# yihua7/NeRF-Texture

Measured on AMD Instinct MI355X. Metric: ray-samples/s (train), higher is better.
Workload: dtype f16

## Files before the change

nerf-texture_amd/csrc/common.hpp:

```cpp
#pragma once

#include <hip/hip_runtime.h>
#include <hip/hip_fp16.h>
#include <stdint.h>

#include <cstdarg>
#include <cstdio>

#include "../../include/nerftex_hip.h"

namespace nerftex {

void set_error(const char* fmt, ...);
void clear_error();

inline hipStream_t as_stream(void* s) { return reinterpret_cast<hipStream_t>(s); }

inline int check_launch(const char* what) {
    hipError_t e = hipGetLastError();
    if (e != hipSuccess) {
        set_error("%s: HIP launch failed: %s", what, hipGetErrorString(e));
        return NERFTEX_ERR_HIP;
    }
    return NERFTEX_OK;
}

#define NERFTEX_HIP_TRY(expr, what)                                                   \
    do {                                                                              \
        hipError_t _e = (expr);                                                       \
        if (_e != hipSuccess) {                                                       \
            ::nerftex::set_error("%s: %s", what, hipGetErrorString(_e));              \
            return NERFTEX_ERR_HIP;                                                   \
        }                                                                             \
    } while (0)

template <typename T>
constexpr T div_up(T a, T b) { return (a + b - 1) / b; }

inline int device_cus() {
    static int cus[16] = {0};
    int dev = 0;
    if (hipGetDevice(&dev) != hipSuccess || dev < 0 || dev >= 16) return 256;
    if (cus[dev] == 0) {
        hipDeviceProp_t prop;
        cus[dev] = (hipGetDeviceProperties(&prop, dev) == hipSuccess && prop.multiProcessorCount > 0) ? prop.multiProcessorCount : 256;
    }
    return cus[dev];
}

enum Knob {
    kKnobGridFwd,
    kKnobGridBwd,
    kKnobGridBwdSweep,
    kKnobGridBwdItems,
    kKnobGridBwdSlice,
    kKnobGridBwdNoMerge,
    kKnobGridBwdProbe,
    kKnobMarch,
    kKnobMarchSerial,
    kKnobFfmlpWgPerCu,
    kKnobFfmlpBwdSplit,
    kKnobMarchLean,
    kKnobFfmlpBwdTr,
    kKnobGridBwdStage,
    kKnobCompositeKeep,
    kKnobCount
};
extern long g_knobs[kKnobCount];
inline long knob(Knob k) { return g_knobs[k]; }

extern int g_profile_mode;
constexpr int kTimeAny = 1, kTimeGrid = 2;
void profile_begin(const char* name, hipStream_t st, int* slot);
void profile_end(hipStream_t st, int slot);
struct KernelTimer {
    hipStream_t st;
    int slot = -1;
    KernelTimer(const char* name, hipStream_t s, int group = kTimeAny) : st(s) {
        if (g_profile_mode == 1 || (g_profile_mode == 2 && group == kTimeGrid)) profile_begin(name, s, &slot);
    }
    ~KernelTimer() { if (slot >= 0) profile_end(st, slot); }
};

using half_t = _Float16;
typedef _Float16 half2_t __attribute__((ext_vector_type(2)));
typedef _Float16 half4_t __attribute__((ext_vector_type(4)));
typedef _Float16 half8_t __attribute__((ext_vector_type(8)));
typedef float float2_t __attribute__((ext_vector_type(2)));
typedef float float4_t __attribute__((ext_vector_type(4)));
typedef float float16_t __attribute__((ext_vector_type(16)));

constexpr int kWave = 64;

__host__ __device__ __forceinline__ uint32_t unit_rows(uint32_t code, uint32_t count) {
    if (!(code >> 31)) return code;
    const uint32_t F = (code >> 24) & 127u, N = code & 0xffffffu;
    const uint32_t q = F * N / (count ? count : 1u);
    return q < F ? F : (q > 8u * F ? 8u * F : q);
}
__device__ __forceinline__ uint32_t live_rows(uint32_t B, const int32_t* __restrict__ units_dev, uint32_t rows_per_unit) {
    if (!units_dev) return B;
    const uint32_t n = (uint32_t)units_dev[0];
    return min(B, n * unit_rows(rows_per_unit, n));
}
__device__ __forceinline__ bool slot_unused(const float* __restrict__ dirs, size_t row) { return dirs[row * 3] > 1e29f; }

}
```

nerf-texture_amd/csrc/raymarching.hip:

```cpp
#include "common.hpp"
#include "step_loss.hpp"
#include "workspace.hpp"

#include <cstdlib>
#include <type_traits>

#pragma clang fp contract(off)

namespace nerftex {
namespace {

constexpr float kSqrt3 = 1.7320508075688772f;
constexpr float kRPi = 0.3183098861837907f;
constexpr uint32_t kBlock = 256;
constexpr uint32_t kRayBlock = 64;

struct Pcg32 {
    uint64_t state, inc;
    static constexpr uint64_t kMult = 0x5851f42d4c957f2dULL;

    __host__ __device__ explicit Pcg32(uint64_t initstate, uint64_t initseq = 1) {
        state = 0;
        inc = (initseq << 1u) | 1u;
        next_uint();
// ... 212 lines not shown
    near_out = near;
    far_out = far;
}

__global__ __launch_bounds__(kBlock) void near_far_kernel(const float* __restrict__ rays_o, const float* __restrict__ rays_d,
                                                          const float* __restrict__ aabb, uint32_t N, float min_near,
                                                          float* __restrict__ nears, float* __restrict__ fars) {
    const uint32_t n = blockIdx.x * blockDim.x + threadIdx.x;
    if (n >= N) return;
    float near, far;
    near_far_of(rays_o, rays_d, aabb, min_near, (size_t)n, near, far);
    nears[n] = near;
    fars[n] = far;
}

__global__ __launch_bounds__(kBlock) void polar_kernel(const float* __restrict__ rays_o, const float* __restrict__ rays_d,
                                                       float radius, uint32_t N, float* __restrict__ coords) {
    const uint32_t n = blockIdx.x * blockDim.x + threadIdx.x;
    if (n >= N) return;
    const float ox = rays_o[3 * (size_t)n], oy = rays_o[3 * (size_t)n + 1], oz = rays_o[3 * (size_t)n + 2];
    const float dx = rays_d[3 * (size_t)n], dy = rays_d[3 * (size_t)n + 1], dz = rays_d[3 * (size_t)n + 2];
    const float A = fmaf(dz, dz, fmaf(dy, dy, dx * dx));
    const float Bh = fmaf(oz, dz, fmaf(oy, dy, ox * dx));
    const float Cc = fmaf(-radius, radius, fmaf(oz, oz, fmaf(oy, oy, ox * ox)));
    const float t = (-Bh + sqrtf(fmaf(Bh, Bh, -(A * Cc)))) / A;
    const float x = fmaf(t, dx, ox), y = fmaf(t, dy, oy), z = fmaf(t, dz, oz);
    const float theta = atan2f(sqrtf(fmaf(z, z, x * x)), y);
    const float phi = atan2f(z, x);
    coords[2 * (size_t)n] = fmaf(2 * theta, kRPi, -1.0f);
    coords[2 * (size_t)n + 1] = phi * kRPi;
}

__global__ __launch_bounds__(kBlock) void morton3D_kernel(const int* __restrict__ coords, uint32_t N, int* __restrict__ indices) {
    const uint32_t n = blockIdx.x * blockDim.x + threadIdx.x;
    if (n >= N) return;
    indices[n] = (int)morton3D((uint32_t)coords[3 * (size_t)n], (uint32_t)coords[3 * (size_t)n + 1], (uint32_t)coords[3 * (size_t)n + 2]);
}

__global__ __launch_bounds__(kBlock) void morton3D_invert_kernel(const int* __restrict__ indices, uint32_t N, int* __restrict__ coords) {
    const uint32_t n = blockIdx.x * blockDim.x + threadIdx.x;
    if (n >= N) return;
    const int ind = indices[n];
    coords[3 * (size_t)n + 0] = (int)morton3D_invert((uint32_t)(ind >> 0));
    coords[3 * (size_t)n + 1] = (int)morton3D_invert((uint32_t)(ind >> 1));
    coords[3 * (size_t)n + 2] = (int)morton3D_invert((uint32_t)(ind >> 2));
}

__global__ __launch_bounds__(kBlock) void packbits_kernel(const float* __restrict__ grid, uint32_t N, float thresh,
                                                          uint8_t* __restrict__ bitfield) {
    const uint32_t n = blockIdx.x * blockDim.x + threadIdx.x;
    if (n >= N) return;
    const float4_t a = *reinterpret_cast<const float4_t*>(grid + (size_t)n * 8);
    const float4_t b = *reinterpret_cast<const float4_t*>(grid + (size_t)n * 8 + 4);
    uint32_t bits = 0;
#pragma unroll
    for (int i = 0; i < 4; i++) {
        bits |= (a[i] > thresh) ? (1u << i) : 0u;
        bits |= (b[i] > thresh) ? (1u << (4 + i)) : 0u;
    }
    bitfield[n] = (uint8_t)bits;
}

__device__ __forceinline__ float ray_t0(const Dda& s, float near, uint32_t perturb, uint32_t n, uint64_t seed) {
    float t0 = near;
    if (perturb) {
        Pcg32 rng(seed);
        rng.advance((uint64_t)n);
        t0 = fmaf(s.dt_min, rng.next_float(), t0);
    }
    return t0;
}

#ifndef NERFTEX_MC_RAYS
#define NERFTEX_MC_RAYS 32
#endif
constexpr uint32_t kMcRays = NERFTEX_MC_RAYS;
static_assert(kRayBlock % kMcRays == 0, "the expand pass adds whole count-pass totals per 64-ray block");
constexpr uint32_t kMcSeg = 128;
constexpr uint32_t kMcSub = 32;
constexpr uint32_t kMcThreads = kMcRays * kMcSub;
constexpr uint32_t kMcPer = kMcSeg / kMcSub;
constexpr uint32_t kMcTPitch = kMcRays + 1;
constexpr uint32_t kMcJPitch = kMcSeg + 4;

template <bool LEAN>
__global__ __launch_bounds__(kMcThreads, LEAN ? 8 : 4) void march_count_parallel_kernel(const float* __restrict__ rays_o, const float* __restrict__ rays_d,
                                                                         const uint8_t* __restrict__ grid, float bound, float dt_gamma,
                                                                         uint32_t max_steps, uint32_t N, uint32_t C, uint32_t H,
                                                                         const float* __restrict__ nears, const float* __restrict__ fars,
                                                                         int* __restrict__ rays, const int* __restrict__ counter,
                                                                         uint32_t* __restrict__ ws, uint32_t perturb, float* __restrict__ tlog,
                                                                         const float* __restrict__ aabb, float min_near,
                                                                         float* __restrict__ nears_w, float* __restrict__ fars_w) {
    __shared__ float s_T[kMcSeg * kMcTPitch];
    __shared__ uint8_t s_jump[kMcRays * kMcJPitch];
    __shared__ uint8_t s_vis[kMcRays * kMcJPitch];
    __shared__ uint32_t s_cnt[kMcRays];
    __shared__ uint32_t s_full[kMcRays];
    __shared__ uint32_t s_base[kMcRays];
    __shared__ uint32_t s_live;

    const uint32_t tid = threadIdx.x;
    const uint32_t own = tid, n_own = blockIdx.x * kMcRays + own;
    const bool owner = tid < kMcRays && n_own < N;
    const uint32_t r2 = tid / kMcSub, sub = tid % kMcSub, n2 = blockIdx.x * kMcRays + r2;
    const bool has2 = n2 < N;
    float near2 = 0.0f, far2 = 0.0f;
    if (has2) {
        if (aabb) near_far_of(rays_o, rays_d, aabb, min_near, (size_t)n2, near2, far2);
        else far2 = fars[n2];
    }
    const Dda s2(rays_o + 3 * (size_t)(has2 ? n2 : 0), rays_d + 3 * (size_t)(has2 ? n2 : 0), bound, dt_gamma, max_steps, C, H, grid, far2);
    float* log_row2 = tlog + (size_t)(has2 ? n2 : 0) * max_steps;

    float t_next = 0.0f, far = 0.0f, pending_tt = 0.0f;
    bool pending = false, done = true;
    uint32_t num = 0;
    if (owner) {
        float near;
        if (aabb) {
            near_far_of(rays_o, rays_d, aabb, min_near, (size_t)n_own, near, far);
            nears_w[n_own] = near;
            fars_w[n_own] = far;
        } else {
            far = fars[n_own];
            near = nears[n_own];
        }
        t_next = ray_t0(s2, near, perturb, n_own, 42);
        done = !(t_next < far);
    }
    const float dt_min = s2.dt_lo, dt_max = s2.dt_max;

    for (;;) {
        if (tid == 0) s_live = 0;
        for (uint32_t i = tid; i < kMcRays * kMcJPitch / 4; i += kMcThreads) reinterpret_cast<uint32_t*>(s_vis)[i] = 0u;
        __syncthreads();
        if (tid < kMcRays) {
            uint32_t cnt = 0;
            if (owner && !done) {
                float t = t_next;
                while (cnt < kMcSeg) {
                    const float t0 = t;
                    const float t1 = t0 + __builtin_amdgcn_fmed3f(t0 * dt_gamma, dt_min, dt_max);
                    const float t2 = t1 + __builtin_amdgcn_fmed3f(t1 * dt_gamma, dt_min, dt_max);
                    const float t3 = t2 + __builtin_amdgcn_fmed3f(t2 * dt_gamma, dt_min, dt_max);
                    s_T[(cnt + 0) * kMcTPitch + own] = t0;
                    s_T[(cnt + 1) * kMcTPitch + own] = t1;
                    s_T[(cnt + 2) * kMcTPitch + own] = t2;
                    s_T[(cnt + 3) * kMcTPitch + own] = t3;
                    if (!(t3 < far)) {
                        cnt += (t0 < far ? 1u : 0u) + (t1 < far ? 1u : 0u) + (t2 < far ? 1u : 0u);
                        t = far;
                        break;
                    }
                    cnt += 4;
                    t = t3 + __builtin_amdgcn_fmed3f(t3 * dt_gamma, dt_min, dt_max);
                }
                t_next = t;
                atomicOr(&s_live, 1u);
            }
            s_cnt[own] = cnt;
            s_full[own] = (owner && !done && cnt == kMcSeg && t_next < far) ? 1u : 0u;
            s_base[own] = num;
        }
        __syncthreads();
        if (s_live == 0) break;

        {
            const uint32_t cnt = s_cnt[r2];
            Dda::Cell cell[kMcPer];
            uint8_t occ_byte[kMcPer];
#pragma unroll
            for (uint32_t i = 0; i < kMcPer; i++) {
                const uint32_t k = sub + kMcSub * i;
                occ_byte[i] = 0;
                cell[i] = Dda::Cell{};
                if (k < cnt) {
                    const uint32_t index = s2.locate(s_T[k * kMcTPitch + r2], cell[i]);
                    occ_byte[i] = grid[index >> 3];
                }
            }
#pragma unroll
            for (uint32_t i = 0; i < kMcPer; i++) {
                const uint32_t k = sub + kMcSub * i;
                if (k < cnt) {
                    uint32_t jump = 0;
                    if (!((occ_byte[i] >> (cell[i].packed >> 29)) & 1u)) {
                        const float t = s_T[k * kMcTPitch + r2];
                        const float tt = s2.exit_of(t, cell[i]);
                        uint32_t j = k + 1;
                        for (;;) {
                            uint32_t c = 0;
#pragma unroll
                            for (uint32_t q = 0; q < 4; q++) c += (j + q < cnt && s_T[(j + q) * kMcTPitch + r2] < tt) ? 1u : 0u;
                            j += c;
                            if (c < 4) break;
                        }
                        jump = j - k;
                    }
                    s_jump[r2 * kMcJPitch + k] = (uint8_t)jump;
                }
            }
        }
        __syncthreads();

        if (owner && !done) {
            const uint32_t cnt = s_cnt[own];
            const bool full = s_full[own] != 0;
            const uint8_t* jr = s_jump + own * kMcJPitch;
            uint8_t* vr = s_vis + own * kMcJPitch;
            uint32_t k = 0;
            if (pending) {
                while (k < cnt && s_T[k * kMcTPitch + own] < pending_tt) k++;
                pending = k == cnt && full;
            }
            uint32_t last_skip = 0xffffffffu;
            while (k < cnt && num < max_steps) {
                const uint32_t j = jr[k];
                const uint32_t sample = j == 0 ? 1u : 0u;
                vr[k] = (uint8_t)sample;
                num += sample;
                last_skip = (j != 0 && k + j == cnt) ? k : last_skip;
                k += j + sample;
            }
            if (full && last_skip != 0xffffffffu && k == cnt && num < max_steps) {
                Dda::Cell c;
                const float t = s_T[last_skip * kMcTPitch + own];
                const Dda so(rays_o + 3 * (size_t)n_own, rays_d + 3 * (size_t)n_own, bound, dt_gamma, max_steps, C, H, grid, far);
                (void)so.locate(t, c);
                pending_tt = so.exit_of(t, c);
                pending = true;
            }
            if (!full || num >= max_steps) done = true;
        }
        __syncthreads();

        {
            uint32_t mine = 0;
            uint32_t flags = 0;
#pragma unroll
            for (uint32_t i = 0; i < kMcPer; i++) {
                const uint32_t k = sub * kMcPer + i;
                const uint32_t v = s_vis[r2 * kMcJPitch + k];
                flags |= v << i;
                mine += v;
            }
            uint32_t incl = mine;
#pragma unroll
            for (int off = 1; off < (int)kMcSub; off <<= 1) {
                const uint32_t o = __shfl_up(incl, off, kMcSub);
                if ((int)sub >= off) incl += o;
            }
            uint32_t at = s_base[r2] + incl - mine;
            if (has2 && flags) {
#pragma unroll
                for (uint32_t i = 0; i < kMcPer; i++)
                    if ((flags >> i) & 1u) log_row2[at++] = s_T[(sub * kMcPer + i) * kMcTPitch + r2];
            }
        }
        __syncthreads();
    }

    if (owner) rays[3 * (size_t)n_own + 2] = (int)num;
    if (tid < kWave) {
        const uint32_t wsum = wave_sum(tid < kMcRays ? num : 0u);
        if (tid == 0) {
            ws[1 + blockIdx.x] = wsum;
            if (blockIdx.x == 0) ws[0] = aabb ? 0u : (uint32_t)counter[0];
        }
    }
}

__global__ __launch_bounds__(kRayBlock) void march_count_kernel(const float* __restrict__ rays_o, const float* __restrict__ rays_d,
                                                             const uint8_t* __restrict__ grid, float bound, float dt_gamma,
                                                             uint32_t max_steps, uint32_t N, uint32_t C, uint32_t H,
                                                             const float* __restrict__ nears, const float* __restrict__ fars,
                                                             int* __restrict__ rays, const int* __restrict__ counter,
                                                             uint32_t* __restrict__ ws, uint32_t perturb, float* __restrict__ tlog) {
    __shared__ uint32_t wave_tot[kRayBlock / kWave];
    const uint32_t n = blockIdx.x * blockDim.x + threadIdx.x;
    uint32_t num_steps = 0;
    if (n < N) {
        const Dda s(rays_o + 3 * (size_t)n, rays_d + 3 * (size_t)n, bound, dt_gamma, max_steps, C, H, grid, fars[n]);
        float t = ray_t0(s, nears[n], perturb, n, 42);
        float x, y, z, dt;
        float* log_row = tlog ? tlog + (size_t)n * max_steps : nullptr;
        while (t < s.far && num_steps < max_steps) {
            if (s.step(t, x, y, z, dt)) {
                if (log_row) log_row[num_steps] = t;
                num_steps++;
                t += dt;
            }
        }
        rays[3 * (size_t)n + 2] = (int)num_steps;
    }
    const uint32_t wsum = wave_sum(num_steps);
    if ((threadIdx.x & (kWave - 1)) == 0) wave_tot[threadIdx.x / kWave] = wsum;
    __syncthreads();
    if (threadIdx.x == 0) {
        uint32_t tot = 0;
#pragma unroll
        for (uint32_t i = 0; i < kRayBlock / kWave; i++) tot += wave_tot[i];
        ws[1 + blockIdx.x] = tot;
        if (blockIdx.x == 0) ws[0] = (uint32_t)counter[0];
    }
}

template <bool WITH_TS>
__global__ __launch_bounds__(kRayBlock) void march_write_kernel(const float* __restrict__ rays_o, const float* __restrict__ rays_d,
                                                             const uint8_t* __restrict__ grid, float bound, float dt_gamma,
                                                             uint32_t max_steps, uint32_t N, uint32_t C, uint32_t H, uint32_t M,
                                                             const float* __restrict__ nears, const float* __restrict__ fars,
                                                             float* __restrict__ xyzs, float* __restrict__ dirs,
                                                             float* __restrict__ deltas, float* __restrict__ rays_ts,
                                                             int* __restrict__ rays, int* __restrict__ counter,
                                                             const uint32_t* __restrict__ ws, uint32_t perturb) {
    __shared__ uint32_t red[kRayBlock / kWave];
    __shared__ uint32_t wave_tot[kRayBlock / kWave];
    const uint32_t n = blockIdx.x * blockDim.x + threadIdx.x;
    const uint32_t lane = threadIdx.x & (kWave - 1), wid = threadIdx.x / kWave;

    uint32_t part = 0;
    for (uint32_t j = threadIdx.x; j < blockIdx.x; j += kRayBlock) part += ws[1 + j];
    part = wave_sum(part);
    if (lane == 0) red[wid] = part;

    const uint32_t num_steps = n < N ? (uint32_t)rays[3 * (size_t)n + 2] : 0u;
    const uint32_t incl = wave_inclusive_scan(num_steps);
    if (lane == kWave - 1) wave_tot[wid] = incl;
    __syncthreads();
    uint32_t before = ws[0];
#pragma unroll
    for (uint32_t i = 0; i < kRayBlock / kWave; i++) {
        before += red[i];
        if (i < wid) before += wave_tot[i];
    }
    const uint32_t point_index = before + incl - num_steps;

    if (blockIdx.x == gridDim.x - 1 && threadIdx.x == kRayBlock - 1) {
        counter[0] = (int)(point_index + num_steps);
        counter[1] = counter[1] + (int)N;
    }
    if (n >= N) return;

    rays[3 * (size_t)n] = (int)n;
    rays[3 * (size_t)n + 1] = (int)point_index;
    if (num_steps == 0) return;
    if (point_index + num_steps >= M) return;
// ... 645 lines not shown
    const float t_old = n < n_alive ? rays_t_old[n] : -1.0f;
    const bool keep = n < n_alive && t_old >= 0;
    const uint64_t mask = __ballot(keep);
    const uint32_t rank = (uint32_t)__popcll(mask & ((1ull << lane) - 1ull));
    if (lane == 0) wave_tot[wid] = (uint32_t)__popcll(mask);
    __syncthreads();
    uint32_t before = ws[0];
    uint32_t block_total = 0;
#pragma unroll
    for (uint32_t i = 0; i < kBlock / kWave; i++) {
        before += red[i];
        if (i < wid) before += wave_tot[i];
        block_total += wave_tot[i];
    }
    if (keep) {
        const uint32_t dst = before + rank;
        rays_alive[dst] = rays_alive_old[n];
        rays_t[dst] = t_old;
    }
    if (blockIdx.x == gridDim.x - 1 && threadIdx.x == 0) {
        uint32_t prior = ws[0];
#pragma unroll
        for (uint32_t i = 0; i < kBlock / kWave; i++) prior += red[i];
        uint32_t survivors = prior + block_total;
        if (steps_done != nullptr) {
            const uint32_t done = steps_done[0];
            if (done >= max_steps) survivors = 0u;
            else steps_done[0] = done + unit_rows(n_step_code, survivors);
        }
        alive_counter[0] = (int)survivors;
        if (host_mirror != nullptr) __hip_atomic_store(host_mirror, (int)survivors, __ATOMIC_RELAXED, __HIP_MEMORY_SCOPE_SYSTEM);
    }
}

inline dim3 grid_for(uint32_t n) { return dim3(div_up(n, kBlock)); }
inline dim3 ray_grid_for(uint32_t n) { return dim3(div_up(n, kRayBlock)); }

__global__ __launch_bounds__(kBlock) void zero_words_kernel(uint32_t* __restrict__ a, size_t na, uint32_t* __restrict__ b, size_t nb) {
    for (size_t i = (size_t)blockIdx.x * kBlock + threadIdx.x; i < na + nb; i += (size_t)gridDim.x * kBlock) {
        if (i < na) a[i] = 0u;
        else b[i - na] = 0u;
    }
}

template <bool WITH_TS>
int march_train_impl(const float* rays_o, const float* rays_d, const uint8_t* grid, float bound, float dt_gamma,
                     uint32_t max_steps, uint32_t N, uint32_t C, uint32_t H, uint32_t M, const float* nears, const float* fars,
                     float* xyzs, float* dirs, float* deltas, float* rays_ts, int32_t* rays, int32_t* counter, uint32_t perturb,
                     void* stream, const float* aabb = nullptr, float min_near = 0.0f) {
    clear_error();
    if (N == 0) return NERFTEX_OK;
    if (C == 0 || C > 16) {
        set_error("march_rays_train: cascade count C=%u out of range", C);
        return NERFTEX_ERR_INVALID;
    }
    const uint32_t nblocks = div_up(N, kRayBlock);
    const size_t head = (sizeof(uint32_t) * (1 + (size_t)div_up(N, kMcRays)) + 255) / 256 * 256;
    const size_t log_bytes = sizeof(float) * (size_t)N * max_steps;
    const long force = knob(kKnobMarch);
    const bool use_log = force ? force == 2 : (log_bytes <= ((size_t)1 << 30));
    char* base = static_cast<char*>(workspace(kWsMarch, head + (use_log ? log_bytes : 0), as_stream(stream)));
    if (!base) return NERFTEX_ERR_HIP;
    uint32_t* ws = reinterpret_cast<uint32_t*>(base);
    float* tlog = use_log ? reinterpret_cast<float*>(base + head) : nullptr;
    hipStream_t st = as_stream(stream);
    const bool parallel_count = use_log && H <= 256 && !knob(kKnobMarchSerial);
    if (aabb && !parallel_count) {
        {
            KernelTimer kt("near_far_kernel", st);
            hipLaunchKernelGGL(near_far_kernel, grid_for(N), dim3(kBlock), 0, st, rays_o, rays_d, aabb, N, min_near, const_cast<float*>(nears),
                               const_cast<float*>(fars));
        }
        {
            KernelTimer kt("zero_words_kernel", st);
            hipLaunchKernelGGL(zero_words_kernel, dim3(1024), dim3(kBlock), 0, st, reinterpret_cast<uint32_t*>(xyzs), (size_t)M * 8,
                               reinterpret_cast<uint32_t*>(counter), (size_t)2);
        }
        int rc0 = check_launch("march_rays_train_fresh(prologue)");
        if (rc0 != NERFTEX_OK) return rc0;
        aabb = nullptr;
    }
    if (parallel_count) {
        KernelTimer kt("march_count_parallel_kernel", st);
        if (knob(kKnobMarchLean))
            hipLaunchKernelGGL(march_count_parallel_kernel<true>, dim3(div_up(N, kMcRays)), dim3(kMcThreads), 0, st, rays_o, rays_d, grid, bound, dt_gamma,
                               max_steps, N, C, H, nears, fars, rays, counter, ws, perturb, tlog, aabb, min_near, const_cast<float*>(nears),
                               const_cast<float*>(fars));
        else
            hipLaunchKernelGGL(march_count_parallel_kernel<false>, dim3(div_up(N, kMcRays)), dim3(kMcThreads), 0, st, rays_o, rays_d, grid, bound, dt_gamma,
                               max_steps, N, C, H, nears, fars, rays, counter, ws, perturb, tlog, aabb, min_near, const_cast<float*>(nears),
                               const_cast<float*>(fars));
    } else {
        KernelTimer kt("march_count_kernel", st);
        hipLaunchKernelGGL(march_count_kernel, dim3(nblocks), dim3(kRayBlock), 0, st, rays_o, rays_d, grid, bound, dt_gamma, max_steps, N,
                           C, H, nears, fars, rays, counter, ws, perturb, tlog);
    }
    int rc = check_launch("march_rays_train(count)");
    if (rc != NERFTEX_OK) return rc;
    if (use_log) {
        {
            KernelTimer kt("march_expand_kernel", st);
            hipLaunchKernelGGL((march_expand_kernel<WITH_TS>), dim3(nblocks), dim3(kExpandThreads), 0, st, rays_o, rays_d, bound, dt_gamma, max_steps, N, C, H, M,
                               nears, xyzs, dirs, deltas, rays_ts, rays, counter, ws, perturb, tlog, parallel_count ? kRayBlock / kMcRays : 1u,
                               parallel_count ? div_up(N, kMcRays) : nblocks, aabb ? 1u : 0u);
        }
        return check_launch("march_rays_train(expand)");
    }
    {
        KernelTimer kt("march_write_kernel", st);
        hipLaunchKernelGGL((march_write_kernel<WITH_TS>), dim3(nblocks), dim3(kRayBlock), 0, st, rays_o, rays_d, grid, bound, dt_gamma,
                           max_steps, N, C, H, M, nears, fars, xyzs, dirs, deltas, rays_ts, rays, counter, ws, perturb);
    }
    return check_launch("march_rays_train(write)");
}

}
}

using namespace nerftex;

extern "C" int nerftex_near_far_from_aabb(const float* rays_o, const float* rays_d, const float* aabb, uint32_t N, float min_near,
                                          float* nears, float* fars, void* stream) {
    clear_error();
    if (N == 0) return NERFTEX_OK;
    {
        KernelTimer kt("near_far_kernel", as_stream(stream));
        hipLaunchKernelGGL(near_far_kernel, grid_for(N), dim3(kBlock), 0, as_stream(stream), rays_o, rays_d, aabb, N, min_near, nears, fars);
    }
    return check_launch("near_far_from_aabb");
}

extern "C" int nerftex_polar_from_ray(const float* rays_o, const float* rays_d, float radius, uint32_t N, float* coords, void* stream) {
    clear_error();
    if (N == 0) return NERFTEX_OK;
    {
        KernelTimer kt("polar_kernel", as_stream(stream));
        hipLaunchKernelGGL(polar_kernel, grid_for(N), dim3(kBlock), 0, as_stream(stream), rays_o, rays_d, radius, N, coords);
    }
    return check_launch("polar_from_ray");
}

extern "C" int nerftex_morton3D(const int32_t* coords, uint32_t N, int32_t* indices, void* stream) {
    clear_error();
    if (N == 0) return NERFTEX_OK;
    {
        KernelTimer kt("morton3D_kernel", as_stream(stream));
        hipLaunchKernelGGL(morton3D_kernel, grid_for(N), dim3(kBlock), 0, as_stream(stream), coords, N, indices);
    }
    return check_launch("morton3D");
}

extern "C" int nerftex_morton3D_invert(const int32_t* indices, uint32_t N, int32_t* coords, void* stream) {
    clear_error();
    if (N == 0) return NERFTEX_OK;
    {
        KernelTimer kt("morton3D_invert_kernel", as_stream(stream));
        hipLaunchKernelGGL(morton3D_invert_kernel, grid_for(N), dim3(kBlock), 0, as_stream(stream), indices, N, coords);
    }
    return check_launch("morton3D_invert");
}

extern "C" int nerftex_packbits(const float* grid, uint32_t N, float density_thresh, uint8_t* bitfield, void* stream) {
    clear_error();
    if (N == 0) return NERFTEX_OK;
    {
        KernelTimer kt("packbits_kernel", as_stream(stream));
        hipLaunchKernelGGL(packbits_kernel, grid_for(N), dim3(kBlock), 0, as_stream(stream), grid, N, density_thresh, bitfield);
    }
    return check_launch("packbits");
}

extern "C" int nerftex_march_rays_train(const float* rays_o, const float* rays_d, const uint8_t* grid, float bound, float dt_gamma,
                                        uint32_t max_steps, uint32_t N, uint32_t C, uint32_t H, uint32_t M, const float* nears,
                                        const float* fars, float* xyzs, float* dirs, float* deltas, int32_t* rays, int32_t* counter,
// ... 296 lines not shown
```

nerf-texture_amd/csrc/runtime.hip:

```cpp
#include "common.hpp"
#include "workspace.hpp"

#include <atomic>

#include <cstdlib>
#include <cstring>
#include <map>
#include <mutex>
#include <string>
#include <vector>

namespace nerftex {

static thread_local char g_err[512] = {0};

void set_error(const char* fmt, ...) {
    va_list ap;
    va_start(ap, fmt);
    vsnprintf(g_err, sizeof(g_err), fmt, ap);
    va_end(ap);
}

void clear_error() { g_err[0] = 0; }

long g_knobs[kKnobCount] = {0};
namespace {
const char* const kKnobNames[kKnobCount] = {"grid_fwd", "grid_bwd", "grid_bwd_sweep", "grid_bwd_items", "grid_bwd_slice", "grid_bwd_nomerge",
                                            "grid_bwd_probe", "march", "march_serial", "ffmlp_wg_per_cu",
                                            "ffmlp_bwd_split", "march_lean", "ffmlp_bwd_tr", "grid_bwd_stage", "composite_keep"};
int knob_index(const char* name, size_t n) {
    for (int k = 0; k < kKnobCount; k++)
        if (strlen(kKnobNames[k]) == n && strncmp(kKnobNames[k], name, n) == 0) return k;
    return -1;
}
struct KnobInit {
    KnobInit() {
        auto env = [](const char* n) { const char* v = getenv(n); return v ? v : ""; };
        const char* v;
        v = env("NERFTEX_GRID_FWD"); g_knobs[kKnobGridFwd] = v[0] == 'p' ? 1 : v[0] == 'l' ? 2 : 0;
        v = env("NERFTEX_GRID_BWD"); g_knobs[kKnobGridBwd] = v[0] == 'a' ? 1 : v[0] == 'o' ? 2 : 0;
        g_knobs[kKnobGridBwdSweep] = env("NERFTEX_GRID_BWD_ALGO")[0] == 's';
        g_knobs[kKnobGridBwdItems] = atol(env("NERFTEX_GRID_BWD_ITEMS"));
        g_knobs[kKnobGridBwdSlice] = atol(env("NERFTEX_GRID_BWD_SLICE"));
        g_knobs[kKnobGridBwdNoMerge] = getenv("NERFTEX_GRID_BWD_NOMERGE") != nullptr;
        v = env("NERFTEX_MARCH"); g_knobs[kKnobMarch] = v[0] == 'r' ? 1 : v[0] == 'l' ? 2 : 0;
        g_knobs[kKnobMarchSerial] = env("NERFTEX_MARCH_COUNT")[0] == 's';
        g_knobs[kKnobFfmlpWgPerCu] = atol(env("NERFTEX_FFMLP_WG_PER_CU"));
        g_knobs[kKnobFfmlpBwdSplit] = env("NERFTEX_FFMLP_BWD")[0] == 's';
        for (const char* p = env("NERFTEX_TUNE"); *p;) {
            const char* eq = strchr(p, '=');
            if (!eq) break;
            const int k = knob_index(p, (size_t)(eq - p));
            if (k >= 0) g_knobs[k] = atol(eq + 1);
            const char* c = strchr(eq, ',');
            if (!c) break;
            p = c + 1;
        }
    }
} g_knob_init;
}

namespace {
constexpr int kMaxDevices = 16;
struct Slot { void* ptr = nullptr; size_t bytes = 0; };
struct SlotSet { Slot slot[kWsSlots]; };
std::map<hipStream_t, SlotSet> g_ws[kMaxDevices];
const hipStream_t kCaptureSet = reinterpret_cast<hipStream_t>(~(uintptr_t)0);
std::vector<void*> g_retired;
std::mutex g_ws_mutex;
}

std::atomic<unsigned> g_ws_touched{0};
thread_local int t_capture_set = 0;

void* workspace(WorkspaceSlot slot, size_t bytes, hipStream_t stream) {
    g_ws_touched.fetch_or(1u << (unsigned)slot, std::memory_order_relaxed);
    int dev = 0;
    if (hipGetDevice(&dev) != hipSuccess || dev < 0 || dev >= kMaxDevices) {
        set_error("workspace: bad device");
        return nullptr;
    }
    hipStreamCaptureStatus cap = hipStreamCaptureStatusNone;
    if (hipStreamIsCapturing(stream, &cap) == hipSuccess && cap != hipStreamCaptureStatusNone)
        stream = reinterpret_cast<hipStream_t>(reinterpret_cast<uintptr_t>(kCaptureSet) - (uintptr_t)t_capture_set);
    std::lock_guard<std::mutex> lock(g_ws_mutex);
    Slot& s = g_ws[dev][stream].slot[slot];
    if (s.bytes < bytes) {
        if (s.ptr) g_retired.push_back(s.ptr);
        s.ptr = nullptr;
        s.bytes = 0;
        size_t want = bytes < (1u << 20) ? (1u << 20) : bytes + bytes / 2;
        hipStreamCaptureMode mode = hipStreamCaptureModeRelaxed;
        (void)hipThreadExchangeStreamCaptureMode(&mode);
        const hipError_t err = hipMalloc(&s.ptr, want);
        (void)hipThreadExchangeStreamCaptureMode(&mode);
        if (err != hipSuccess) {
            set_error("workspace: hipMalloc(%zu) failed", want);
            s.ptr = nullptr;
            return nullptr;
        }
        s.bytes = want;
        static const int poison = [] { const char* v = getenv("NERFTEX_POISON_WORKSPACE"); return v && *v ? atoi(v) : -1; }();
        if (poison >= 0) {
            (void)hipThreadExchangeStreamCaptureMode(&mode);
            (void)hipMemset(s.ptr, poison & 255, want);
            (void)hipThreadExchangeStreamCaptureMode(&mode);
        }
    }
    return s.ptr;
}

bool peek_workspace(int slot, hipStream_t stream, void** ptr, size_t* bytes) {
// ... 147 lines not shown
```

Baseline: 909.8 million.

## Parallelize march count skip-chain walk with pointer jumping across ray sub-lanes

Replaces the serial per-ray owner walk over the jump table in the parallel march-count kernel with a pointer-jumping pass run by the 32 lanes assigned to each ray, synchronized at wave level. The pending-skip offset is computed with a shuffle reduction, cell exit times are carried in registers instead of being re-located, and sample offsets come from ballot/popcount. This removes a serial loop and two block barriers per segment. In exchange it adds several rounds of LDS traffic per segment, and it adds a probe knob that can skip phases for timing.

```diff
diff --git a/nerf-texture_amd/csrc/common.hpp b/nerf-texture_amd/csrc/common.hpp
--- a/nerf-texture_amd/csrc/common.hpp
+++ b/nerf-texture_amd/csrc/common.hpp
@@ -64,6 +64,7 @@
     kKnobFfmlpBwdTr,
     kKnobGridBwdStage,
     kKnobCompositeKeep,
+    kKnobMarchCountProbe,
     kKnobCount
 };
 extern long g_knobs[kKnobCount];
diff --git a/nerf-texture_amd/csrc/raymarching.hip b/nerf-texture_amd/csrc/raymarching.hip
--- a/nerf-texture_amd/csrc/raymarching.hip
+++ b/nerf-texture_amd/csrc/raymarching.hip
@@ -318,6 +318,15 @@
 constexpr uint32_t kMcPer = kMcSeg / kMcSub;
 constexpr uint32_t kMcTPitch = kMcRays + 1;
 constexpr uint32_t kMcJPitch = kMcSeg + 4;
+constexpr uint32_t kMcRounds = 7;
+static_assert((1u << kMcRounds) >= kMcSeg && kMcSeg <= 255, "a path is covered by the rounds; member indices fit a byte");
+static_assert(kMcSub == 32 && kWave == 64, "a ray is one half of a wave in phases 2-4 (ballot halves, wave-level ordering of LDS)");
+
+__device__ __forceinline__ void wave_lds_order() {
+    __builtin_amdgcn_fence(__ATOMIC_RELEASE, "wavefront");
+    __builtin_amdgcn_wave_barrier();
+    __builtin_amdgcn_fence(__ATOMIC_ACQUIRE, "wavefront");
+}
 
 template <bool LEAN>
 __global__ __launch_bounds__(kMcThreads, LEAN ? 8 : 4) void march_count_parallel_kernel(const float* __restrict__ rays_o, const float* __restrict__ rays_d,
@@ -327,19 +336,21 @@
                                                                          int* __restrict__ rays, const int* __restrict__ counter,
                                                                          uint32_t* __restrict__ ws, uint32_t perturb, float* __restrict__ tlog,
                                                                          const float* __restrict__ aabb, float min_near,
-                                                                         float* __restrict__ nears_w, float* __restrict__ fars_w) {
+                                                                         float* __restrict__ nears_w, float* __restrict__ fars_w, const uint32_t probe) {
     __shared__ float s_T[kMcSeg * kMcTPitch];
-    __shared__ uint8_t s_jump[kMcRays * kMcJPitch];
-    __shared__ uint8_t s_vis[kMcRays * kMcJPitch];
+    __shared__ uint32_t s_next[kMcRays * kMcJPitch / 4];
+    __shared__ uint32_t s_mark[kMcRays * kMcJPitch / 4];
     __shared__ uint32_t s_cnt[kMcRays];
     __shared__ uint32_t s_full[kMcRays];
-    __shared__ uint32_t s_base[kMcRays];
+    __shared__ uint32_t s_num[kMcRays];
+    __shared__ uint32_t s_done[kMcRays];
     __shared__ uint32_t s_live;
 
     const uint32_t tid = threadIdx.x;
     const uint32_t own = tid, n_own = blockIdx.x * kMcRays + own;
     const bool owner = tid < kMcRays && n_own < N;
     const uint32_t r2 = tid / kMcSub, sub = tid % kMcSub, n2 = blockIdx.x * kMcRays + r2;
+    const uint32_t half = tid & 32u;
     const bool has2 = n2 < N;
     float near2 = 0.0f, far2 = 0.0f;
     if (has2) {
@@ -348,62 +359,88 @@
     }
     const Dda s2(rays_o + 3 * (size_t)(has2 ? n2 : 0), rays_d + 3 * (size_t)(has2 ? n2 : 0), bound, dt_gamma, max_steps, C, H, grid, far2);
     float* log_row2 = tlog + (size_t)(has2 ? n2 : 0) * max_steps;
-
-    float t_next = 0.0f, far = 0.0f, pending_tt = 0.0f;
-    bool pending = false, done = true;
+    uint32_t* const next_w = s_next + r2 * (kMcJPitch / 4) + sub;
+    uint32_t* const mark_w = s_mark + r2 * (kMcJPitch / 4) + sub;
+    uint8_t* const next_b = reinterpret_cast<uint8_t*>(s_next + r2 * (kMcJPitch / 4));
+    uint8_t* const mark_b = reinterpret_cast<uint8_t*>(s_mark + r2 * (kMcJPitch / 4));
+
+    float t_next = 0.0f, far = 0.0f;
+    if (tid < kMcRays) {
+        bool done = true;
+        if (owner) {
+            float near;
+            if (aabb) {
+                near_far_of(rays_o, rays_d, aabb, min_near, (size_t)n_own, near, far);
+                nears_w[n_own] = near;
+                fars_w[n_own] = far;
+            } else {
+                far = fars[n_own];
+                near = nears[n_own];
+            }
+            t_next = ray_t0(s2, near, perturb, n_own, 42);
+            done = !(t_next < far);
+        }
+        s_done[own] = done ? 1u : 0u;
+        s_num[own] = 0u;
+    }
+    const float dt_min = s2.dt_lo, dt_max = s2.dt_max;
+    float pending_tt = 0.0f;
+    bool pending = false;
     uint32_t num = 0;
-    if (owner) {
-        float near;
-        if (aabb) {
-            near_far_of(rays_o, rays_d, aabb, min_near, (size_t)n_own, near, far);
-            nears_w[n_own] = near;
-            fars_w[n_own] = far;
-        } else {
-            far = fars[n_own];
-            near = nears[n_own];
-        }
-        t_next = ray_t0(s2, near, perturb, n_own, 42);
-        done = !(t_next < far);
-    }
-    const float dt_min = s2.dt_lo, dt_max = s2.dt_max;
 
     for (;;) {
         if (tid == 0) s_live = 0;
-        for (uint32_t i = tid; i < kMcRays * kMcJPitch / 4; i += kMcThreads) reinterpret_cast<uint32_t*>(s_vis)[i] = 0u;
-        __syncthreads();
         if (tid < kMcRays) {
             uint32_t cnt = 0;
-            if (owner && !done) {
+            const bool run = owner && s_done[own] == 0;
+            if (run) {
                 float t = t_next;
-                while (cnt < kMcSeg) {
+#pragma unroll 2
+                for (uint32_t k = 0; k < kMcSeg; k += 4) {
                     const float t0 = t;
                     const float t1 = t0 + __builtin_amdgcn_fmed3f(t0 * dt_gamma, dt_min, dt_max);
                     const float t2 = t1 + __builtin_amdgcn_fmed3f(t1 * dt_gamma, dt_min, dt_max);
                     const float t3 = t2 + __builtin_amdgcn_fmed3f(t2 * dt_gamma, dt_min, dt_max);
-                    s_T[(cnt + 0) * kMcTPitch + own] = t0;
-                    s_T[(cnt + 1) * kMcTPitch + own] = t1;
-                    s_T[(cnt + 2) * kMcTPitch + own] = t2;
-                    s_T[(cnt + 3) * kMcTPitch + own] = t3;
-                    if (!(t3 < far)) {
-                        cnt += (t0 < far ? 1u : 0u) + (t1 < far ? 1u : 0u) + (t2 < far ? 1u : 0u);
-                        t = far;
-                        break;
-                    }
-                    cnt += 4;
+                    s_T[(k + 0) * kMcTPitch + own] = t0;
+                    s_T[(k + 1) * kMcTPitch + own] = t1;
+                    s_T[(k + 2) * kMcTPitch + own] = t2;
+                    s_T[(k + 3) * kMcTPitch + own] = t3;
+                    cnt += (t0 < far ? 1u : 0u) + (t1 < far ? 1u : 0u) + (t2 < far ? 1u : 0u) + (t3 < far ? 1u : 0u);
                     t = t3 + __builtin_amdgcn_fmed3f(t3 * dt_gamma, dt_min, dt_max);
+                    if (!__any(t < far ? 1 : 0)) break;
                 }
                 t_next = t;
                 atomicOr(&s_live, 1u);
             }
             s_cnt[own] = cnt;
-            s_full[own] = (owner && !done && cnt == kMcSeg && t_next < far) ? 1u : 0u;
-            s_base[own] = num;
+            s_full[own] = (run && cnt == kMcSeg && t_next < far) ? 1u : 0u;
         }
         __syncthreads();
         if (s_live == 0) break;
-
+        const uint32_t cnt = s_cnt[r2];
+        const bool full = s_full[r2] != 0;
+        if (probe == 1) {
+            if (sub == 0) s_done[r2] = full ? 0u : 1u;
+            __syncthreads();
+            continue;
+        }
+
+        uint32_t jmp[kMcPer];
+        float ext[kMcPer];
         {
-            const uint32_t cnt = s_cnt[r2];
+            uint32_t k0 = 0;
+            if (__any(pending ? 1 : 0)) {
+                uint32_t c = 0;
+#pragma unroll
+                for (uint32_t i = 0; i < kMcPer; i++) {
+                    const uint32_t k = sub + kMcSub * i;
+                    c += (pending && k < cnt && s_T[k * kMcTPitch + r2] < pending_tt) ? 1u : 0u;
+                }
+#pragma unroll
+                for (int off = (int)kMcSub / 2; off > 0; off >>= 1) c += __shfl_xor(c, off, kMcSub);
+                k0 = c;
+                pending = pending && k0 == cnt && full;
+            }
             Dda::Cell cell[kMcPer];
             uint8_t occ_byte[kMcPer];
 #pragma unroll
@@ -419,6 +456,9 @@
 #pragma unroll
             for (uint32_t i = 0; i < kMcPer; i++) {
                 const uint32_t k = sub + kMcSub * i;
+                jmp[i] = 0;
+                ext[i] = 0.0f;
+                uint32_t to = cnt;
                 if (k < cnt) {
                     uint32_t jump = 0;
                     if (!((occ_byte[i] >> (cell[i].packed >> 29)) & 1u)) {
@@ -433,73 +473,76 @@
                             if (c < 4) break;
                         }
                         jump = j - k;
+                        ext[i] = tt;
                     }
-                    s_jump[r2 * kMcJPitch + k] = (uint8_t)jump;
+                    jmp[i] = jump;
+                    to = k + (jump ? jump : 1u);
                 }
+                next_b[k] = (uint8_t)to;
+                mark_b[k] = (k < cnt && k == k0) ? 1 : 0;
             }
+            if (sub == 0) next_b[kMcSeg] = (uint8_t)kMcSeg;
+        }
+        if (probe == 2) {
+            if (sub == 0) s_done[r2] = full ? 0u : 1u;
+            __syncthreads();
+            continue;
+        }
+
+        wave_lds_order();
+        for (uint32_t round = 0; round < kMcRounds; round++) {
+            const uint32_t nx = *next_w, mk = *mark_w;
+            bool more = false;
+#pragma unroll
+            for (uint32_t i = 0; i < 4; i++) more = more || (((mk >> (8 * i)) & 0xffu) != 0 && ((nx >> (8 * i)) & 0xffu) != cnt);
+            if (!__any(more ? 1 : 0)) break;
+            uint32_t nn = 0;
+#pragma unroll
+            for (uint32_t i = 0; i < 4; i++) nn |= (uint32_t)next_b[(nx >> (8 * i)) & 0xffu] << (8 * i);
+            wave_lds_order();
+            *next_w = nn;
+#pragma unroll
+            for (uint32_t i = 0; i < 4; i++)
+                if ((mk >> (8 * i)) & 0xffu) mark_b[(nx >> (8 * i)) & 0xffu] = 1;
+            wave_lds_order();
+        }
+
+        uint32_t at = num;
+        bool last_skip = false;
+        float last_ext = 0.0f;
+#pragma unroll
+        for (uint32_t i = 0; i < kMcPer; i++) {
+            const uint32_t k = sub + kMcSub * i;
+            const bool on = k < cnt && mark_b[k] != 0;
+            const bool vis = on && jmp[i] == 0;
+            const uint32_t mine = (uint32_t)(__ballot(vis ? 1 : 0) >> half);
+            const uint32_t rank = at + (uint32_t)__popc(mine & ((1u << sub) - 1u));
+            if (vis && rank < max_steps && probe != 3) log_row2[rank] = s_T[k * kMcTPitch + r2];
+            at += (uint32_t)__popc(mine);
+            if (on && jmp[i] != 0 && k + jmp[i] == cnt) {
+                last_skip = true;
+                last_ext = ext[i];
+            }
+        }
+        const bool capped = at >= max_steps;
+        num = capped ? max_steps : at;
+        const uint32_t holder = (uint32_t)(__ballot(last_skip ? 1 : 0) >> half);
+        const float carried = __shfl(last_ext, holder ? __ffs((int)holder) - 1 : 0, kMcSub);
+        if (holder != 0 && full && !capped) {
+            pending_tt = carried;
+            pending = true;
+        }
+        if (sub == 0) {
+            s_num[r2] = num;
+            s_done[r2] = (!full || capped) ? 1u : 0u;
         }
         __syncthreads();
-
-        if (owner && !done) {
-            const uint32_t cnt = s_cnt[own];
-            const bool full = s_full[own] != 0;
-            const uint8_t* jr = s_jump + own * kMcJPitch;
-            uint8_t* vr = s_vis + own * kMcJPitch;
-            uint32_t k = 0;
-            if (pending) {
-                while (k < cnt && s_T[k * kMcTPitch + own] < pending_tt) k++;
-                pending = k == cnt && full;
-            }
-            uint32_t last_skip = 0xffffffffu;
-            while (k < cnt && num < max_steps) {
-                const uint32_t j = jr[k];
-                const uint32_t sample = j == 0 ? 1u : 0u;
-                vr[k] = (uint8_t)sample;
-                num += sample;
-                last_skip = (j != 0 && k + j == cnt) ? k : last_skip;
-                k += j + sample;
-            }
-            if (full && last_skip != 0xffffffffu && k == cnt && num < max_steps) {
-                Dda::Cell c;
-                const float t = s_T[last_skip * kMcTPitch + own];
-                const Dda so(rays_o + 3 * (size_t)n_own, rays_d + 3 * (size_t)n_own, bound, dt_gamma, max_steps, C, H, grid, far);
-                (void)so.locate(t, c);
-                pending_tt = so.exit_of(t, c);
-                pending = true;
-            }
-            if (!full || num >= max_steps) done = true;
-        }
-        __syncthreads();
-
-        {
-            uint32_t mine = 0;
-            uint32_t flags = 0;
-#pragma unroll
-            for (uint32_t i = 0; i < kMcPer; i++) {
-                const uint32_t k = sub * kMcPer + i;
-                const uint32_t v = s_vis[r2 * kMcJPitch + k];
-                flags |= v << i;
-                mine += v;
-            }
-            uint32_t incl = mine;
-#pragma unroll
-            for (int off = 1; off < (int)kMcSub; off <<= 1) {
-                const uint32_t o = __shfl_up(incl, off, kMcSub);
-                if ((int)sub >= off) incl += o;
-            }
-            uint32_t at = s_base[r2] + incl - mine;
-            if (has2 && flags) {
-#pragma unroll
-                for (uint32_t i = 0; i < kMcPer; i++)
-                    if ((flags >> i) & 1u) log_row2[at++] = s_T[(sub * kMcPer + i) * kMcTPitch + r2];
-            }
-        }
-        __syncthreads();
-    }
-
-    if (owner) rays[3 * (size_t)n_own + 2] = (int)num;
+    }
+
+    const uint32_t num_own = tid < kMcRays ? s_num[tid] : 0u;
+    if (owner) rays[3 * (size_t)n_own + 2] = (int)num_own;
     if (tid < kWave) {
-        const uint32_t wsum = wave_sum(tid < kMcRays ? num : 0u);
+        const uint32_t wsum = wave_sum(num_own);
         if (tid == 0) {
             ws[1 + blockIdx.x] = wsum;
             if (blockIdx.x == 0) ws[0] = aabb ? 0u : (uint32_t)counter[0];
@@ -1311,14 +1354,15 @@
     }
     if (parallel_count) {
         KernelTimer kt("march_count_parallel_kernel", st);
+        const uint32_t mc_probe = (uint32_t)knob(kKnobMarchCountProbe);
         if (knob(kKnobMarchLean))
             hipLaunchKernelGGL(march_count_parallel_kernel<true>, dim3(div_up(N, kMcRays)), dim3(kMcThreads), 0, st, rays_o, rays_d, grid, bound, dt_gamma,
                                max_steps, N, C, H, nears, fars, rays, counter, ws, perturb, tlog, aabb, min_near, const_cast<float*>(nears),
-                               const_cast<float*>(fars));
+                               const_cast<float*>(fars), mc_probe);
         else
             hipLaunchKernelGGL(march_count_parallel_kernel<false>, dim3(div_up(N, kMcRays)), dim3(kMcThreads), 0, st, rays_o, rays_d, grid, bound, dt_gamma,
                                max_steps, N, C, H, nears, fars, rays, counter, ws, perturb, tlog, aabb, min_near, const_cast<float*>(nears),
-                               const_cast<float*>(fars));
+                               const_cast<float*>(fars), mc_probe);
     } else {
         KernelTimer kt("march_count_kernel", st);
         hipLaunchKernelGGL(march_count_kernel, dim3(nblocks), dim3(kRayBlock), 0, st, rays_o, rays_d, grid, bound, dt_gamma, max_steps, N,
diff --git a/nerf-texture_amd/csrc/runtime.hip b/nerf-texture_amd/csrc/runtime.hip
--- a/nerf-texture_amd/csrc/runtime.hip
+++ b/nerf-texture_amd/csrc/runtime.hip
@@ -27,7 +27,7 @@
 namespace {
 const char* const kKnobNames[kKnobCount] = {"grid_fwd", "grid_bwd", "grid_bwd_sweep", "grid_bwd_items", "grid_bwd_slice", "grid_bwd_nomerge",
                                             "grid_bwd_probe", "march", "march_serial", "ffmlp_wg_per_cu",
-                                            "ffmlp_bwd_split", "march_lean", "ffmlp_bwd_tr", "grid_bwd_stage", "composite_keep"};
+                                            "ffmlp_bwd_split", "march_lean", "ffmlp_bwd_tr", "grid_bwd_stage", "composite_keep", "march_count_probe"};
 int knob_index(const char* name, size_t n) {
     for (int k = 0; k < kKnobCount; k++)
         if (strlen(kKnobNames[k]) == n && strncmp(kKnobNames[k], name, n) == 0) return k;
```

Result: faster. 928.5 million (median of 6 runs) (+2.1%).
